# StefanSko/mcmc-db

Hardware: AMD Instinct MI355X
Metric: validated param-draws/sec (higher is better)
Workload: dtype f64; 1 GPU; single posteriordb-shaped model, 4x10000x100 synthetic draws per GPU (BASELINE config 1; AR(1) chains, ties and a shifted chain; SURVEY 8(d) C1); layout=pcn, statistics=mean,std,q5,q50,q95,split_rhat,ess_bulk,ess_tail

## Files before the change

mcmc-db_amd/csrc/mcr_kernels.hpp:

```cpp
#pragma once
#include <type_traits>
#include "mcr_device.hpp"
#include "mcr_sortnet.h"

namespace mcr {

enum ResField {
    R_MEAN = 0, R_STD, R_MEDIAN, R_RHAT, R_RHAT_BULK, R_RHAT_TAIL, R_ESS_BULK, R_ESS_TAIL,
    R_LAG_BULK, R_LAG_TAIL, R_BAD, R_Q0
};

#ifndef MCR_WCOMB
#define MCR_WCOMB 1
#endif
constexpr bool kWriteCombine = MCR_WCOMB != 0;

struct QArgs {
    int nq;
    i64 lo[32];
    double g[32];
    const void* xt = nullptr;
    int xf32 = 0;
};

// ... 194 lines not shown
        const bool sw = k[b] < k[a];                                        \
        const double lo = sw ? k[b] : k[a], hi = sw ? k[a] : k[b];          \
        const u32 ilo = sw ? ix[b] : ix[a], ihi = sw ? ix[a] : ix[b];       \
        k[a] = lo; k[b] = hi; ix[a] = ilo; ix[b] = ihi;                     \
    }
    if constexpr (VT == 16) { MCR_NET16(MCR_CE) } else { MCR_NET8(MCR_CE) }
#undef MCR_CE
}

#ifndef MCR_TILE_DPP_LEVELS
#define MCR_TILE_DPP_LEVELS 3
#endif

__device__ __forceinline__ u32 select_by_mask(u32 a, u32 b, unsigned long long m)
{
    u32 r;
    asm("v_cndmask_b32_e64 %0, %1, %2, %3" : "=v"(r) : "v"(a), "v"(b), "s"(m));
    return r;
}
__device__ __forceinline__ double select_by_mask(double a, double b, unsigned long long m)
{
    return __hiloint2double((int)select_by_mask((u32)__double2hiint(a), (u32)__double2hiint(b), m),
                            (int)select_by_mask((u32)__double2loint(a), (u32)__double2loint(b), m));
}

template <int CTRL, bool MIRROR, unsigned long long MIN_LANES>
__device__ __forceinline__ void lane_pair_stage(double (&k)[16], u32 (&ix)[16])
{
    auto exchange = [](double& own, u32& own_i, double o, u32 oi) {
        const unsigned long long lt = __builtin_amdgcn_ballot_w64(o < own), gt = __builtin_amdgcn_ballot_w64(own < o);
        const unsigned long long take = (lt & MIN_LANES) | (gt & ~MIN_LANES);
        own = select_by_mask(own, o, take);
        own_i = select_by_mask(own_i, oi, take);
    };
#pragma unroll
    for (int r = 0; r < (MIRROR ? 8 : 16); ++r) {
        const int s = MIRROR ? 15 - r : r;
        const double o_r = dpp_f64<CTRL>(k[s]);
        const u32 oi_r = dpp_u32<CTRL>(ix[s]);
        if (MIRROR) {
            const double o_s = dpp_f64<CTRL>(k[r]);
            const u32 oi_s = dpp_u32<CTRL>(ix[r]);
            exchange(k[s], ix[s], o_s, oi_s);
        }
        exchange(k[r], ix[r], o_r, oi_r);
    }
}

__device__ __forceinline__ void lane_bitonic_merge16(double (&k)[16], u32 (&ix)[16])
{
#define MCR_CE(a, b)                                                        \
    {                                                                       \
        const bool sw = k[b] < k[a];                                        \
        const double lo = sw ? k[b] : k[a], hi = sw ? k[a] : k[b];          \
        const u32 ilo = sw ? ix[b] : ix[a], ihi = sw ? ix[a] : ix[b];       \
        k[a] = lo; k[b] = hi; ix[a] = ilo; ix[b] = ihi;                     \
    }
    MCR_BITONIC16(MCR_CE)
#undef MCR_CE
}

__device__ __forceinline__ void lane_merge_levels_16_to_64(double (&k)[16], u32 (&ix)[16])
{
    constexpr unsigned long long kEvenLanes = 0x5555555555555555ull, kLowPairs = 0x3333333333333333ull;
    lane_pair_stage<0xB1, true, kEvenLanes>(k, ix);
    lane_bitonic_merge16(k, ix);
    lane_pair_stage<0x1B, true, kLowPairs>(k, ix);
    lane_pair_stage<0xB1, false, kEvenLanes>(k, ix);
    lane_bitonic_merge16(k, ix);
#if MCR_TILE_DPP_LEVELS >= 3
    constexpr unsigned long long kLowQuads = 0x0F0F0F0F0F0F0F0Full;
    lane_pair_stage<0x141, true, kLowQuads>(k, ix);
    lane_pair_stage<0x4E, false, kLowPairs>(k, ix);
    lane_pair_stage<0xB1, false, kEvenLanes>(k, ix);
    lane_bitonic_merge16(k, ix);
#endif
}

template <int VT>
__device__ __forceinline__ void serial_merge(const double* skey, int a0, int na, int b0, int nb, int ai,
                                             int bi, int nout, double (&k)[VT], int (&src)[VT])
{
    int pa = a0 + ai, pb = b0 + bi;
    const int ea = a0 + na, eb = b0 + nb;
    double ak = skey[pos16(pa)], bk = skey[pos16(pb)];
#pragma unroll
    for (int i = 0; i < VT; ++i) {
        if (i < nout) {
            const bool takeA = (pb >= eb) | ((pa < ea) & !(bk < ak));
            k[i] = takeA ? ak : bk;
            src[i] = takeA ? pa : pb;
            pa += takeA ? 1 : 0;
            pb += takeA ? 0 : 1;
            const int pn = takeA ? pa : pb;
            const double nv = skey[pos16(pn)];
            ak = takeA ? nv : ak;
            bk = takeA ? bk : nv;
        } else {
            src[i] = 0;
        }
    }
}

#ifndef MCR_TILE_REC
#define MCR_TILE_REC 1
#endif
#if MCR_TILE_REC == 0
#define MCR_TILE_PAIRS_INLINE __forceinline__
#else
#define MCR_TILE_PAIRS_INLINE __noinline__
#endif

template <typename IdxT> constexpr size_t sort_lds_bytes(int T) { return (size_t)T * (8 + sizeof(IdxT)); }

template <int NT, int VT, typename IdxT, typename XT>
__device__ MCR_TILE_PAIRS_INLINE void tile_sort_pairs(const XT* __restrict__ X, i64 M,
                                                      double* __restrict__ keys, IdxT* __restrict__ idx,
                                                      double* __restrict__ part, int ntiles,
                                                      double* __restrict__ samp)
{
    constexpr int T = NT * VT;
    extern __shared__ __attribute__((aligned(16))) char smem[];
    double* skey = reinterpret_cast<double*>(smem);
    IdxT* sidx = reinterpret_cast<IdxT*>(skey + T);
    double* red = skey;

    const int tid = threadIdx.x, tile = blockIdx.x;
    const i64 p = blockIdx.y;
    const i64 base = (i64)tile * T;
    const int count = (int)((M - base < (i64)T) ? M - base : (i64)T);
    const XT* src = X + p * M + base;

    const bool full = count == T;
    double k[VT];
    u32 ix[VT];
    double bad = 0.0;
    auto load = [&](auto full_c) {
        constexpr bool FULL = decltype(full_c)::value;
#pragma unroll
        for (int i = 0; i < VT; ++i) {
            const int e = i * NT + tid;
            const bool live = FULL || e < count;
            const double v = (double)src[FULL ? e : min(e, count - 1)];
            k[i] = live ? v : INFINITY;
            ix[i] = live ? (u32)(base + e) : 0xFFFFFFFFu;
            bad += (live && !isfinite(v)) ? 1.0 : 0.0;
        }
    };
    if (full) load(std::true_type{}); else load(std::false_type{});
    thread_sort<VT>(k, ix);
    constexpr bool kLaneLevels = MCR_TILE_DPP_LEVELS >= 2 && VT == 16;
    if constexpr (kLaneLevels) lane_merge_levels_16_to_64(k, ix);
#pragma unroll
    for (int i = 0; i < VT; ++i) {
        const int e = tid * VT + i;
        skey[pos16(e)] = k[i];
        sidx[posi(e)] = (IdxT)ix[i];
    }
    __syncthreads();

    for (int coop = kLaneLevels ? (MCR_TILE_DPP_LEVELS >= 3 ? 16 : 8) : 2; coop <= NT; coop <<= 1) {
        const int first = tid & ~(coop - 1);
        const int run = VT * (coop >> 1);
        const int a0 = first * VT, b0 = a0 + run;
        const int diag = VT * (tid - first);
        auto A = [&](int i) { return skey[pos16(a0 + i)]; };
        auto B = [&](int j) { return skey[pos16(b0 + j)]; };
        const int ai = merge_path32(A, run, B, run, diag);
        int srcs[VT];
        serial_merge<VT>(skey, a0, run, b0, run, ai, diag - ai, VT, k, srcs);
#pragma unroll
        for (int i = 0; i < VT; ++i) ix[i] = sidx[posi(srcs[i])];
        __syncthreads();
#pragma unroll
        for (int i = 0; i < VT; ++i) {
            const int e = tid * VT + i;
            skey[pos16(e)] = k[i];
            sidx[posi(e)] = (IdxT)ix[i];
        }
        __syncthreads();
    }

    auto write_out = [&](auto full_c) {
        constexpr bool FULL = decltype(full_c)::value;
#pragma nounroll
        for (int e = tid; e < (FULL ? T : count); e += NT) {
            keys[p * M + base + e] = skey[pos16(e)];
            idx[p * M + base + e] = sidx[posi(e)];
        }
    };
    if (full) write_out(std::true_type{}); else write_out(std::false_type{});
    if (samp != nullptr && tid < T / 64) {
        const int e = 64 * tid + 63;
        samp[(p * ntiles + tile) * (T / 64) + tid] = (e < count) ? skey[pos16(e)] : INFINITY;
    }
    __syncthreads();
    double s1 = 0.0, s2 = 0.0, e1 = 0.0, mt = 0.0;
    auto moments = [&](auto full_c) {
        constexpr bool FULL = decltype(full_c)::value;
        const int nlive = count - tid * VT;
#pragma unroll
        for (int i = 0; i < VT; ++i) s1 += (FULL || i < nlive) ? k[i] : 0.0;
        s1 = block_sum<NT>(s1, red);
        mt = s1 / (double)count;
#pragma unroll
        for (int i = 0; i < VT; ++i) { const double d = (FULL || i < nlive) ? k[i] - mt : 0.0; s2 = fma(d, d, s2); e1 += d; }
    };
    if (full) moments(std::true_type{}); else moments(std::false_type{});
    block_sum3<NT>(s2, e1, bad, red);
    if (tid == 0) store_slice_moments(part + (p * ntiles + tile) * kMomRec, mt, e1, s2, bad, (double)count);
}

#ifndef MCR_TILE_REC_MINMAX
#define MCR_TILE_REC_MINMAX 1
#endif
template <typename R> __device__ __forceinline__ R rec_pad();
template <> __device__ __forceinline__ u64 rec_pad<u64>() { return kRecPad; }
template <> __device__ __forceinline__ double rec_pad<double>() { return INFINITY; }

__device__ __forceinline__ void rec_ce(u64& a, u64& b)
{
    const bool sw = b < a;
    const u64 lo = sw ? b : a, hi = sw ? a : b;
    a = lo; b = hi;
}
__device__ __forceinline__ void rec_ce(double& a, double& b)
{
#if MCR_TILE_REC_MINMAX
    double lo, hi;
    asm("v_min_f64 %0, %1, %2" : "=v"(lo) : "v"(a), "v"(b));
    asm("v_max_f64 %0, %1, %2" : "=v"(hi) : "v"(a), "v"(b));
    a = lo; b = hi;
#else
    const bool sw = b < a;
    const double lo = sw ? b : a, hi = sw ? a : b;
    a = lo; b = hi;
#endif
}

template <int VT, typename R>
__device__ __forceinline__ void thread_sort_rec(R (&r)[VT])
{
    static_assert(VT == 16 || VT == 8, "sorting networks exist for 16 and 8 items per lane");
#define MCR_CE(a, b) rec_ce(r[a], r[b]);
    if constexpr (VT == 16) { MCR_NET16(MCR_CE) } else { MCR_NET8(MCR_CE) }
#undef MCR_CE
}

template <int CTRL>
__device__ __forceinline__ u64 dpp_rec(u64 v)
{
    return ((u64)dpp_u32<CTRL>((u32)(v >> 32)) << 32) | (u64)dpp_u32<CTRL>((u32)v);
}
template <int CTRL>
__device__ __forceinline__ double dpp_rec(double v) { return dpp_f64<CTRL>(v); }
__device__ __forceinline__ u64 select_by_mask(u64 a, u64 b, unsigned long long m)
{
    return ((u64)select_by_mask((u32)(a >> 32), (u32)(b >> 32), m) << 32) | (u64)select_by_mask((u32)a, (u32)b, m);
}

template <int CTRL, bool MIRROR, unsigned long long MIN_LANES, typename R>
__device__ __forceinline__ void lane_pair_stage_rec(R (&r)[16])
{
    auto exchange = [](R& own, R o) {
        const unsigned long long lt = __builtin_amdgcn_ballot_w64(o < own), gt = __builtin_amdgcn_ballot_w64(own < o);
        own = select_by_mask(own, o, (lt & MIN_LANES) | (gt & ~MIN_LANES));
    };
#pragma unroll
    for (int i = 0; i < (MIRROR ? 8 : 16); ++i) {
        const int s = MIRROR ? 15 - i : i;
        const R o_i = dpp_rec<CTRL>(r[s]);
        if (MIRROR) {
            const R o_s = dpp_rec<CTRL>(r[i]);
            exchange(r[s], o_s);
        }
        exchange(r[i], o_i);
    }
}

template <typename R>
__device__ __forceinline__ void lane_bitonic_merge16_rec(R (&r)[16])
{
#define MCR_CE(a, b) rec_ce(r[a], r[b]);
    MCR_BITONIC16(MCR_CE)
#undef MCR_CE
}

template <typename R>
__device__ __forceinline__ void lane_merge_levels_rec(R (&r)[16])
{
    constexpr unsigned long long kEvenLanes = 0x5555555555555555ull, kLowPairs = 0x3333333333333333ull,
                                 kLowQuads = 0x0F0F0F0F0F0F0F0Full;
    lane_pair_stage_rec<0xB1, true, kEvenLanes>(r);
    lane_bitonic_merge16_rec(r);
    lane_pair_stage_rec<0x1B, true, kLowPairs>(r);
    lane_pair_stage_rec<0xB1, false, kEvenLanes>(r);
    lane_bitonic_merge16_rec(r);
    lane_pair_stage_rec<0x141, true, kLowQuads>(r);
    lane_pair_stage_rec<0x4E, false, kLowPairs>(r);
    lane_pair_stage_rec<0xB1, false, kEvenLanes>(r);
    lane_bitonic_merge16_rec(r);
}

template <int VT, int LIM = 0, typename R>
__device__ __forceinline__ void serial_merge_rec(const R* srec, int a0, int na, int b0, int nb, int ai, int bi,
                                                 int nout, R (&out)[VT])
{
    int pa = a0 + ai, pb = b0 + bi;
    const int ea = a0 + na, eb = b0 + nb;
    auto slot = [](int e) { return pos16(LIM > 0 ? min(e, LIM) : e); };
    R ar = srec[slot(pa)], br = srec[slot(pb)];
#pragma unroll
    for (int i = 0; i < VT; ++i) {
        if (i < nout) {
            const bool takeA = (pb >= eb) | ((pa < ea) & !(br < ar));
            out[i] = takeA ? ar : br;
            pa += takeA ? 1 : 0;
            pb += takeA ? 0 : 1;
            const int pn = takeA ? pa : pb;
            const R nv = srec[slot(pn)];
            ar = takeA ? nv : ar;
            br = takeA ? br : nv;
        } else {
            out[i] = rec_pad<R>();
        }
    }
}

template <int NT, int VT, typename IdxT, typename XT>
__global__ __launch_bounds__(NT) __attribute__((amdgpu_waves_per_eu(4))) void k_tile_sort(const XT* __restrict__ X, i64 M,
                                                  double* __restrict__ keys, IdxT* __restrict__ idx,
                                                  double* __restrict__ part, int ntiles,
                                                  double* __restrict__ samp, unsigned* __restrict__ fallbacks)
{
#if MCR_TILE_REC == 0
    tile_sort_pairs<NT, VT, IdxT, XT>(X, M, keys, idx, part, ntiles, samp);
#else
    constexpr int T = NT * VT;
    constexpr u32 kSlotMask = 0xFFFu;
    static_assert(T <= 4096, "a record has 12 bits for the tile slot");
    extern __shared__ __attribute__((aligned(16))) char smem[];
    double* srec = reinterpret_cast<double*>(smem);
    unsigned short* slow = reinterpret_cast<unsigned short*>(srec + T);
    IdxT* sidx = reinterpret_cast<IdxT*>(srec + T);
    double* red = srec;

    const int tid = threadIdx.x, tile = blockIdx.x;
    const i64 p = blockIdx.y;
    const i64 base = (i64)tile * T;
    const int count = (int)((M - base < (i64)T) ? M - base : (i64)T);
    const XT* src = X + p * M + base;
    const bool full = count == T;
    const int nlive = count - tid * VT;

    double r[VT];
    double bad = 0.0;
    auto load = [&](auto full_c) {
        constexpr bool FULL = decltype(full_c)::value;
        XT v[VT];
#pragma unroll
        for (int i = 0; i < VT; ++i) {
            const int e = i * NT + tid;
            v[i] = src[FULL ? e : min(e, count - 1)];
        }
#pragma unroll
        for (int i = 0; i < VT; ++i) {
            const int e = i * NT + tid;
            const bool live = FULL || e < count;
            const double d = (double)v[i];
            const bool fin = isfinite(d);
            bad += (live && !fin) ? 1.0 : 0.0;
            const u32 lo = (u32)__double2loint(d), hi = (u32)__double2hiint(d);
            if (live) slow[e] = (unsigned short)(lo & kSlotMask);
            const double rec = __hiloint2double((int)(fin ? hi : 0u), (int)((lo & ~kSlotMask) | (u32)e));
            r[i] = live ? rec : INFINITY;
        }
    };
    if (full) load(std::true_type{}); else load(std::false_type{});
    thread_sort_rec<VT>(r);
    static_assert(MCR_TILE_DPP_LEVELS == 0 || MCR_TILE_DPP_LEVELS >= 3,
                  "the record sort has all three register levels or none: build MCR_TILE_DPP_LEVELS=2 with MCR_TILE_REC=0");
    constexpr bool kLaneLevels = MCR_TILE_DPP_LEVELS >= 3 && VT == 16;
    if constexpr (kLaneLevels) lane_merge_levels_rec(r);
#pragma unroll
    for (int i = 0; i < VT; ++i) srec[pos16(tid * VT + i)] = r[i];
    __syncthreads();
    for (int coop = kLaneLevels ? 16 : 2; coop <= NT; coop <<= 1) {
        const int first = tid & ~(coop - 1);
        const int run = VT * (coop >> 1);
        const int a0 = first * VT, b0 = a0 + run;
        const int diag = VT * (tid - first);
        auto A = [&](int i) { return srec[pos16(a0 + i)]; };
        auto B = [&](int j) { return srec[pos16(b0 + j)]; };
        const int ai = merge_path32(A, run, B, run, diag);
        serial_merge_rec<VT>(srec, a0, run, b0, run, ai, diag - ai, VT, r);
        __syncthreads();
        if (coop < NT) {
#pragma unroll
            for (int i = 0; i < VT; ++i) srec[pos16(tid * VT + i)] = r[i];
            __syncthreads();
        }
    }

    double k[VT];
    u32 slot[VT];
    bool viol = false;
    auto rebuild = [&](auto full_c) {
        constexpr bool FULL = decltype(full_c)::value;
#pragma unroll
        for (int i = 0; i < VT; ++i) {
            const u32 lo = (u32)__double2loint(r[i]);
            slot[i] = lo & kSlotMask;
            const double key = __hiloint2double(__double2hiint(r[i]), (int)((lo & ~kSlotMask) | (u32)slow[slot[i]]));
            k[i] = (FULL || i < nlive) ? key : INFINITY;
        }
    };
    if (full) rebuild(std::true_type{}); else rebuild(std::false_type{});
#pragma unroll
    for (int i = 0; i + 1 < VT; ++i) viol |= k[i + 1] < k[i];
    constexpr int NW = NT / kWave;
    const int lane = tid & (kWave - 1), wave = tid / kWave;
    const double next_first = dpp_f64<0x130>(k[0]);
    viol |= lane + 1 < kWave && next_first < k[VT - 1];
    int* wflag = reinterpret_cast<int*>(srec + 2 * NW);
    const bool wave_viol = __builtin_amdgcn_ballot_w64(viol) != 0;
    if (lane == 0) { srec[wave] = k[0]; wflag[wave] = wave_viol ? 1 : 0; }
    if (lane == kWave - 1) srec[NW + wave] = k[VT - 1];
    __syncthreads();
    bool fall = MCR_TILE_REC == 2;
#pragma unroll
    for (int w = 0; w < NW; ++w) {
        fall |= wflag[w] != 0;
        if (w + 1 < NW) fall |= srec[w + 1] < srec[NW + w];
    }
    __syncthreads();
    if (fall) {
        if (tid == 0 && fallbacks != nullptr) atomicAdd(fallbacks, 1u);
        tile_sort_pairs<NT, VT, IdxT, XT>(X, M, keys, idx, part, ntiles, samp);
        return;
    }
#pragma unroll
    for (int i = 0; i < VT; ++i) {
        srec[pos16(tid * VT + i)] = k[i];
        sidx[posi(tid * VT + i)] = (IdxT)((u32)base + slot[i]);
    }
    __syncthreads();

    auto write_out = [&](auto full_c) {
        constexpr bool FULL = decltype(full_c)::value;
#pragma nounroll
        for (int e = tid; e < (FULL ? T : count); e += NT) {
            keys[p * M + base + e] = srec[pos16(e)];
            idx[p * M + base + e] = sidx[posi(e)];
        }
    };
    if (full) write_out(std::true_type{}); else write_out(std::false_type{});
    if (samp != nullptr && tid < T / 64) {
        const int e = 64 * tid + 63;
        samp[(p * ntiles + tile) * (T / 64) + tid] = (e < count) ? srec[pos16(e)] : INFINITY;
    }
    __syncthreads();
    double s1 = 0.0, s2 = 0.0, e1 = 0.0, mt = 0.0;
    auto moments = [&](auto full_c) {
        constexpr bool FULL = decltype(full_c)::value;
#pragma unroll
        for (int i = 0; i < VT; ++i) s1 += (FULL || i < nlive) ? k[i] : 0.0;
        s1 = block_sum<NT>(s1, red);
        mt = s1 / (double)count;
#pragma unroll
        for (int i = 0; i < VT; ++i) { const double d = (FULL || i < nlive) ? k[i] - mt : 0.0; s2 = fma(d, d, s2); e1 += d; }
    };
    if (full) moments(std::true_type{}); else moments(std::false_type{});
    block_sum3<NT>(s2, e1, bad, red);
    if (tid == 0) store_slice_moments(part + (p * ntiles + tile) * kMomRec, mt, e1, s2, bad, (double)count);
#endif
}

template <int NT, int VT>
__device__ __forceinline__ void scatter_codes_by_line(u32* __restrict__ zrow, i64 M, int total, const u32 (&hcode)[VT],
                                                      const u32 (&hpos)[VT], u32* cnt_code, unsigned short* spos, u32* swt)
{
    constexpr int kMaxLines = 2048, PER = kMaxLines / NT > 0 ? kMaxLines / NT : 1;
    static_assert(NT * PER >= kMaxLines, "every line counter has an owner in the scan");
    const int tid = threadIdx.x;
    const int nlines = (int)((M + 31) >> 5);
    u32* scnt = cnt_code;
    u32* scode = cnt_code + 2112;
    __syncthreads();
    for (int i = tid; i <= nlines; i += NT) scnt[i] = 0u;
    __syncthreads();
    u32 rk[VT];
#pragma unroll
    for (int i = 0; i < VT; ++i) rk[i] = (tid * VT + i < total) ? atomicAdd(&scnt[hpos[i] >> 5], 1u) : 0u;
    __syncthreads();
    {
        u32 c[PER], tsum = 0;
#pragma unroll
        for (int j = 0; j < PER; ++j) { const int q = tid * PER + j; c[j] = (q < nlines) ? scnt[q] : 0u; tsum += c[j]; }
        u32 wtot;
        const u32 wex = wave_excl_scan_u32(tsum, wtot);
        if ((tid & 63) == 0) swt[tid >> 6] = wtot;
        __syncthreads();
        u32 base = wex;
        for (int w = 0; w < (tid >> 6); ++w) base += swt[w];
#pragma unroll
        for (int j = 0; j < PER; ++j) { const int q = tid * PER + j; if (q < nlines) scnt[q] = base; base += c[j]; }
    }
    __syncthreads();
#pragma unroll
    for (int i = 0; i < VT; ++i) {
        if (tid * VT + i < total) {
            const u32 slot = min(scnt[hpos[i] >> 5] + rk[i], (u32)(NT * VT - 1));
            scode[slot] = hcode[i];
            spos[slot] = (unsigned short)hpos[i];
        }
    }
    __syncthreads();
    for (int e = tid; e < total; e += NT) zrow[spos[e]] = scode[e];
}

template <int NT, int VT, class KF>
__device__ __forceinline__ void block_tie_runs(KF key_at, int total, int* wsh, int (&rs)[VT], int (&re)[VT])
{
    constexpr int NW = NT / kWave;
    const int tid = threadIdx.x, lane = tid & 63, w = tid >> 6;
    const int base = tid * VT;
    bool h[VT];
    auto prev = key_at((base > 0 && base - 1 < total) ? base - 1 : 0);
    int cur = -1, first = 0x7fffffff;
#pragma unroll
    for (int i = 0; i < VT; ++i) {
        const int g = base + i;
        const auto kv = key_at(g < total ? g : 0);
        h[i] = (g == 0) || (g >= total) || (prev != kv);
        if (h[i]) { cur = g; if (first == 0x7fffffff) first = g; }
        rs[i] = cur;
        prev = kv;
    }
    int exL, exR;
    const int incl = wave_prefix_max(cur, exL);
    const int rinc = wave_suffix_min(first, exR);
    __syncthreads();
    if (lane == 63) wsh[w] = incl;
    if (lane == 0) wsh[NW + w] = rinc;
    __syncthreads();
    int carryL = -1, carryR = total;
#pragma unroll
    for (int ww = 0; ww < NW; ++ww) {
        if (ww < w) carryL = max(carryL, wsh[ww]);
        if (ww > w) carryR = min(carryR, wsh[NW + ww]);
    }
    carryL = max(carryL, exL);
    carryR = min(carryR, exR);
    if (carryR > total) carryR = total;
    int nxt = carryR;
#pragma unroll
    for (int i = VT - 1; i >= 0; --i) {
        re[i] = nxt;
        if (h[i]) nxt = base + i;
        if (rs[i] < 0) rs[i] = carryL;
    }
    __syncthreads();
}

__device__ __forceinline__ bool sign_bit_set(double v) { return __double_as_longlong(v) < 0; }
__device__ __forceinline__ bool sign_bit_set(float v) { return __float_as_int(v) < 0; }
template <typename T>
__device__ __noinline__ unsigned wave_zero_signs(const T* __restrict__ x, i64 M, i64 t0, i64 t1)
{
    constexpr int U = 8;
    const int lane = threadIdx.x & 63;
    i64 seen = 0, t = (t0 >= 0) ? t0 : t1;
    unsigned out = 0;
    for (i64 b = 0; b < M; b += 64 * U) {
        T v[U];
#pragma unroll
        for (int u = 0; u < U; ++u) {
            const i64 i = b + u * 64 + lane;
            v[u] = (i < M) ? x[i] : (T)1;
        }
        i64 c = 0;
#pragma unroll
        for (int u = 0; u < U; ++u) c += (i64)__popcll(__ballot(v[u] == (T)0));
        if (seen + c <= t) { seen += c; continue; }
#pragma unroll
        for (int u = 0; u < U; ++u) {
            const unsigned long long zm = __ballot(v[u] == (T)0), nm = __ballot(v[u] == (T)0 && sign_bit_set(v[u]));
            const i64 cu = (i64)__popcll(zm);
            while (seen + cu > t) {
                unsigned long long m = zm;
                for (i64 j = seen; j < t; ++j) m &= m - 1;
                const bool neg = (nm & m & (~m + 1ull)) != 0;
                if (t == t1) return out | (neg ? 2u : 0u);
                out |= neg ? 1u : 0u;
                t = t1;
            }
            seen += cu;
        }
    }
    return out;
}

template <typename KT>
__device__ __forceinline__ i64 wave_order_stats(const KT* __restrict__ k, i64 M, const QArgs& q, bool write,
                                                double* __restrict__ res, i64 P, i64 p, double& med_out)
{
#pragma clang fp contract(off)
    const int lane = threadIdx.x & 63;
    if (write && lane < q.nq) {
        const int j = lane;
        const i64 lo = q.lo[j], hi = (lo + 1 < M) ? lo + 1 : M - 1;
        const double a = sorted_key(k, lo), b = sorted_key(k, hi), d = b - a, g = q.g[j];
        res[(R_Q0 + j) * P + p] = (g >= 0.5) ? b - d * (1.0 - g) : a + d * g;
    }
    const double below = (M >= 2) ? sorted_key(k, M / 2 - 1) : -INFINITY, at = sorted_key(k, M / 2);
    double med = (M & 1) ? at : (below + at) / 2.0;
    const bool zero_med = write && q.xt != nullptr && at == 0.0 && ((M & 1) || below == 0.0);
    if (write && lane == 0 && !zero_med) res[R_MEDIAN * P + p] = med;
    i64 lo = 0, hi = M;
    if (below < med && !(at < med)) {
        if (!zero_med) { med_out = med; return M / 2; }
        lo = hi = M / 2;
    }
    while (lo < hi) {
        const i64 step = (hi - lo + 63) / 64;
        const i64 pos = lo + step * (lane + 1) - 1;
        const bool less = (pos < hi) && (sorted_key(k, pos) < med);
        const i64 cnt = (i64)__popcll(__ballot(less));
        const i64 nhi = lo + step * (cnt + 1) - 1;
        lo += step * cnt;
        hi = (nhi < hi) ? nhi : hi;
    }
    if (zero_med) {
        const i64 r = M / 2 - lo;
        const i64 t0 = (M & 1) ? -1 : r - 1;
        const unsigned sg = q.xf32 ? wave_zero_signs(reinterpret_cast<const float*>(q.xt) + p * M, M, t0, r)
                                   : wave_zero_signs(reinterpret_cast<const double*>(q.xt) + p * M, M, t0, r);
        const bool neg = (M & 1) ? (sg & 2u) != 0 : sg == 3u;
        med = neg ? -0.0 : 0.0;
        if (lane == 0) res[R_MEDIAN * P + p] = med;
    }
    med_out = med;
    return lo;
}

template <int NT, int VT, bool FOLD, typename IdxT, typename KT = double>
__global__ __launch_bounds__(NT) void k_merge(const KT* __restrict__ kin, const IdxT* __restrict__ iin,
                                              double* __restrict__ kout, IdxT* __restrict__ iout, i64 M,
                                              i64 R, double* __restrict__ res, i64 P,
                                              QArgs q, u32* __restrict__ z, const i64* __restrict__ split_in)
{
    constexpr int OBS = NT * VT;
    constexpr int OB = FOLD ? OBS - 64 : OBS;
    extern __shared__ __attribute__((aligned(16))) char smem[];
    double* skey = reinterpret_cast<double*>(smem);
    IdxT* sidx = reinterpret_cast<IdxT*>(skey + OBS);
    i64* sh = FOLD ? reinterpret_cast<i64*>(skey + OB) : reinterpret_cast<i64*>(sidx + OBS);

    const int tid = threadIdx.x;
    i64 p = blockIdx.y;
    int blk = blockIdx.x;
    if (FOLD) {
        if (!xcd_map(P, (int)((M + OB - 1) / OB), p, blk)) return;
    }
    const i64 o0 = (i64)blk * OB;
    if (o0 >= M) return;
    const KT* kp = kin + p * M;
    const IdxT* ip = iin + p * M;
    auto KEY = [&](i64 g) -> double { return sorted_key(kp, g); };
    auto POS = [&](i64 g) -> u32 {
        if constexpr (sizeof(KT) == 8 && !__is_same(KT, double)) return (u32)kp[g]; else return (u32)ip[g];
    };

    i64 abase, na, bbase, nb, d0;
    double med = 0.0;
    if (!FOLD) {
        const i64 pb = (o0 / (2 * R)) * (2 * R);
        abase = pb;
        na = (M - pb < R) ? M - pb : R;
        bbase = pb + na;
        nb = (M - bbase < R) ? M - bbase : R;
        d0 = o0 - pb;
    } else {
        if (split_in != nullptr) {
            if (tid == 0) { sh[0] = split_in[p]; reinterpret_cast<double*>(sh)[1] = res[R_MEDIAN * P + p]; }
        } else if (tid < 64) {
            double m_;
            const i64 s_ = wave_order_stats(kp, M, q, blk == 0, res, P, p, m_);
            if (tid == 0) { sh[0] = s_; reinterpret_cast<double*>(sh)[1] = m_; }
        }
        __syncthreads();
        const i64 s = sh[0];
        med = reinterpret_cast<double*>(sh)[1];
        __syncthreads();
        abase = s - 1;
        na = s;
        bbase = s;
        nb = M - s;
        d0 = o0;
    }
    const i64 tot = na + nb;
    const i64 d1 = (d0 + OB < tot) ? d0 + OB : tot;
// ... 583 lines not shown
```

mcmc-db_amd/csrc/mcr_sort32.hpp:

```cpp
#pragma once
#include "mcr_kernels.hpp"

namespace mcr {

__device__ __forceinline__ u32 rec_key(u64 r) { return (u32)(r >> 32); }
__device__ __forceinline__ u32 rec_pos(u64 r) { return (u32)r; }


constexpr size_t rec_lds_bytes(int T) { return (size_t)(T + 2) * 8; }

template <int NT, int VT>
__global__ __launch_bounds__(NT) void k_tile_sort32(const float* __restrict__ X, i64 M, u64* __restrict__ recs,
                                                    double* __restrict__ part, int ntiles, double* __restrict__ samp)
{
    constexpr int T = NT * VT;
    extern __shared__ __attribute__((aligned(16))) char smem[];
    u64* srec = reinterpret_cast<u64*>(smem);
    double* red = reinterpret_cast<double*>(smem);

    const int tid = threadIdx.x, tile = blockIdx.x;
    const i64 p = blockIdx.y;
    const i64 base = (i64)tile * T;
    const int count = (int)((M - base < (i64)T) ? M - base : (i64)T);
    const float* src = X + p * M + base;

    const bool full = count == T;
    u64 r[VT];
    double bad = 0.0;
    auto load = [&](auto full_c) {
        constexpr bool FULL = decltype(full_c)::value;
#pragma unroll
        for (int i = 0; i < VT; ++i) {
            const int e = i * NT + tid;
            const bool live = FULL || e < count;
            const float v = src[FULL ? e : min(e, count - 1)];
            bad += (live && !isfinite(v)) ? 1.0 : 0.0;
            r[i] = live ? (((u64)f32_key(v) << 32) | (u64)(u32)(base + e)) : kRecPad;
        }
    };
    if (full) load(std::true_type{}); else load(std::false_type{});
    thread_sort_rec<VT>(r);
    constexpr bool kLaneLevels = MCR_TILE_DPP_LEVELS >= 3 && VT == 16;
    if constexpr (kLaneLevels) lane_merge_levels_rec(r);
#pragma unroll
    for (int i = 0; i < VT; ++i) srec[pos16(tid * VT + i)] = r[i];
    __syncthreads();

    for (int coop = kLaneLevels ? 16 : 2; coop <= NT; coop <<= 1) {
        const int first = tid & ~(coop - 1);
        const int run = VT * (coop >> 1);
        const int a0 = first * VT, b0 = a0 + run;
        const int diag = VT * (tid - first);
        auto A = [&](int i) { return srec[pos16(a0 + i)]; };
        auto B = [&](int j) { return srec[pos16(b0 + j)]; };
        const int ai = merge_path32(A, run, B, run, diag);
        serial_merge_rec<VT, T - 1>(srec, a0, run, b0, run, ai, diag - ai, VT, r);
        __syncthreads();
#pragma unroll
        for (int i = 0; i < VT; ++i) srec[pos16(tid * VT + i)] = r[i];
        __syncthreads();
    }
    auto write_out = [&](auto full_c) {
        constexpr bool FULL = decltype(full_c)::value;
#pragma nounroll
        for (int e = tid; e < (FULL ? T : count); e += NT) recs[p * M + base + e] = srec[pos16(e)];
    };
    if (full) write_out(std::true_type{}); else write_out(std::false_type{});
    if (samp != nullptr && tid < T / 64) {
        const int e = 64 * tid + 63;
        samp[(p * ntiles + tile) * (T / 64) + tid] = (e < count) ? key_value(rec_key(srec[pos16(e)])) : INFINITY;
    }
    __syncthreads();
    double s1 = 0.0, s2 = 0.0, e1 = 0.0, mt = 0.0;
    auto moments = [&](auto full_c) {
        constexpr bool FULL = decltype(full_c)::value;
        const int nlive = count - tid * VT;
#pragma unroll
        for (int i = 0; i < VT; ++i) s1 += (FULL || i < nlive) ? key_value(rec_key(r[i])) : 0.0;
        s1 = block_sum<NT>(s1, red);
        mt = s1 / (double)count;
#pragma unroll
        for (int i = 0; i < VT; ++i) { const double d = (FULL || i < nlive) ? key_value(rec_key(r[i])) - mt : 0.0; s2 = fma(d, d, s2); e1 += d; }
    };
    if (full) moments(std::true_type{}); else moments(std::false_type{});
    block_sum3<NT>(s2, e1, bad, red);
    if (tid == 0) store_slice_moments(part + (p * ntiles + tile) * kMomRec, mt, e1, s2, bad, (double)count);
}

template <int NT, int VT>
__global__ __launch_bounds__(NT) void k_merge32(const u64* __restrict__ rin, u64* __restrict__ rout, i64 M, i64 R)
{
    constexpr int OB = NT * VT;
    extern __shared__ __attribute__((aligned(16))) char smem[];
    u64* srec = reinterpret_cast<u64*>(smem);
    __shared__ i64 sh[2];
    const int tid = threadIdx.x;
    const i64 p = blockIdx.y;
    const i64 o0 = (i64)blockIdx.x * OB;
    if (o0 >= M) return;
    const u64* rp = rin + p * M;
    const i64 pb = (o0 / (2 * R)) * (2 * R);
    const i64 abase = pb, na = (M - pb < R) ? M - pb : R;
    const i64 bbase = pb + na, nb = (M - bbase < R) ? M - bbase : R;
    const i64 d0 = o0 - pb, tot = na + nb;
    const i64 d1 = (d0 + OB < tot) ? d0 + OB : tot;
    auto GA = [&](i64 i) { return rp[abase + i]; };
    auto GB = [&](i64 j) { return rp[bbase + j]; };
    if (tid < 64) { const i64 r0 = merge_path_wave(GA, na, GB, nb, d0); if (tid == 0) sh[0] = r0; }
    else if (tid < 128) { const i64 r1 = merge_path_wave(GA, na, GB, nb, d1); if (tid == 64) sh[1] = r1; }
    __syncthreads();
    const i64 ai0 = sh[0], ai1 = sh[1], bi0 = d0 - ai0;
    const int ca = (int)(ai1 - ai0), cb = (int)((d1 - ai1) - bi0);
    const int total = ca + cb;
    {
        u64 gr[VT];
#pragma unroll
        for (int j = 0; j < VT; ++j) {
            const int e = j * NT + tid;
            const i64 g = (e < ca) ? abase + ai0 + e : bbase + bi0 + (e - ca);
            gr[j] = rp[(e < total) ? g : 0];
        }
#pragma unroll
        for (int j = 0; j < VT; ++j) {
            const int e = j * NT + tid;
            if (e < total) srec[pos16(e)] = gr[j];
        }
    }
    __syncthreads();
    const int diag = (tid * VT < total) ? tid * VT : total;
    const int nout = (total - diag < VT) ? total - diag : VT;
    auto A = [&](int i) { return srec[pos16(i)]; };
    auto B = [&](int j) { return srec[pos16(ca + j)]; };
    const int ai = merge_path32(A, ca, B, cb, diag);
    u64 r[VT];
    serial_merge_rec<VT>(srec, 0, ca, ca, cb, ai, diag - ai, nout, r);
    __syncthreads();
#pragma unroll
    for (int i = 0; i < VT; ++i)
        if (i < nout) srec[pos16(diag + i)] = r[i];
    __syncthreads();
    for (int e = tid; e < total; e += NT) rout[p * M + o0 + e] = srec[pos16(e)];
}

template <int NT, int VT>
__global__ __launch_bounds__(NT) void k_bucket_merge32(const u64* __restrict__ rin, u64* __restrict__ rout, i64 M,
                                                       int k, int B, const u32* __restrict__ cut,
                                                       const u32* __restrict__ boff, u32* __restrict__ z, i64 P, i64 R)
{
    constexpr int T = NT * VT;
    static_assert(T == 4096, "the partition bound of k_splitters assumes 4096-slot buckets");
    extern __shared__ __attribute__((aligned(16))) char smem[];
    u64* srec = reinterpret_cast<u64*>(smem);
    int* sst = reinterpret_cast<int*>(srec + T + 2);
    int* spl = sst + kBkLen;
    int* sps = sst + kBkSrc;
    int* sext = sst + kBkExt;
    i64* sedge = reinterpret_cast<i64*>(sst + kBkEdge);
    u64* sne = reinterpret_cast<u64*>(sst + kBkNext);
    static_assert(2 * (NT / kWave) <= 4 * kMaxBucketTiles, "the tie-run scratch takes the neighbours' place");

    const int tid = threadIdx.x;
    i64 p;
    int b;
    if (!xcd_map(P, B, p, b)) return;
    const u64* rp = rin + p * M;
    const u32* c0 = cut + (p * (B + 1) + b) * k;
    const u32* c1 = c0 + k;
    if (k < 1 || k > kMaxBucketTiles) return;
    if (tid < kWave) bucket_piece_table(c0, c1, k, sst, spl, sps);
    __syncthreads();
    const int padded = sst[k];
    const int total = (int)(boff[p * (B + 1) + b + 1] - boff[p * (B + 1) + b]);
    const i64 obase = boff[p * (B + 1) + b];
    if (padded > T - 64 || total < 0 || total > padded || obase + total > M) return;
    const int ne_lane = tid - (T - 64 - (VT - 1) * NT);
    bool ne_there = false;
    i64 ne_g = 0;
    if (ne_lane >= 0) ne_g = bucket_neighbour(ne_lane, k, R, M, spl, sps, ne_there);
    const bool is_ne = ne_lane >= 0 && ne_lane < 2 * k;
    u64 ne = 0;
    {
        const int lane = tid & 63, wv = tid >> 6;
        u32 my_g = 0; int my_n = 0;
        if ((lane & 15) < VT) {
            const int e0 = (lane & 15) * NT + 64 * wv + 16 * (lane >> 4);
            if (e0 < padded) {
                int t = 0;
#pragma unroll
                for (int step = 8; step > 0; step >>= 1)
                    if (t + step < k && e0 >= sst[t + step]) t += step;
                const int o = e0 - sst[t];
                my_n = spl[t] - o;
                my_g = (u32)((i64)t * R) + (u32)sps[t] + (u32)o;
            }
        }
        u64 gr[VT];
#pragma unroll
        for (int j = 0; j < VT; ++j) {
            const int within = lane & 15;
            const u32 g0 = (u32)row_lane((int)my_g, j);
            const int n = row_lane(my_n, j);
            const bool live = within < n;
            i64 g = live ? (i64)(g0 + (u32)within) : 0;
            if (j == VT - 1) g = is_ne ? ne_g : g;
            const u64 r = rp[g];
            gr[j] = live ? r : kRecPad;
            if (j == VT - 1) ne = r;
        }
#pragma unroll
        for (int j = 0; j < VT; ++j) {
            const int e = j * NT + tid;
            if (e < padded) srec[pos16(e)] = gr[j];
        }
    }
    if (is_ne) sne[ne_lane] = ne_there ? (u64)rec_key(ne) : ~0ull;
    wait_loads();
    __syncthreads();
    const int chunk0 = tid * VT;
    int mypiece = 0;
#pragma unroll
    for (int step = 8; step > 0; step >>= 1)
        if (mypiece + step < k && chunk0 >= sst[mypiece + step]) mypiece += step;
    for (int w = 1; w < k; w <<= 1) {
        u64 r[VT];
        bool moved = false;
        if (chunk0 < padded) {
            const int ra = mypiece & ~(2 * w - 1);
            const int a0 = sst[ra];
            const int a1 = sst[(ra + w < k) ? ra + w : k];
            const int b1 = sst[(ra + 2 * w < k) ? ra + 2 * w : k];
            const int na = a1 - a0, nb = b1 - a1, diag = chunk0 - a0;
            moved = nb > 0;
            if (moved) {
                auto A = [&](int i) { return srec[pos16(a0 + i)]; };
                auto Bf = [&](int j) { return srec[pos16(a1 + j)]; };
                const int ai = merge_path32(A, na, Bf, nb, diag);
                serial_merge_rec<VT>(srec, a0, na, a1, nb, ai, diag - ai, VT, r);
            }
        }
        __syncthreads();
        if (moved) {
#pragma unroll
            for (int i = 0; i < VT; ++i) srec[pos16(chunk0 + i)] = r[i];
        }
        __syncthreads();
    }
    for (int e = tid; e < total; e += NT) rout[p * M + obase + e] = srec[pos16(e)];
    if (z == nullptr || total == 0) return;
    if (tid < 4) sedge[tid] = 0;
    const u32 kfirst = rec_key(srec[pos16(0)]), klast = rec_key(srec[pos16(total - 1)]);
    if (tid < kWave) {
        const int t = (tid < k) ? tid : k - 1;
        const bool e0 = tid < k && sne[t] == (u64)kfirst;
        const bool e1 = tid < k && sne[k + t] == (u64)klast;
        const bool a0 = __ballot(e0) != 0, a1 = __ballot(e1) != 0;
        if (tid == 0) { sext[0] = a0; sext[1] = a1; }
    }
    __syncthreads();
    const bool ext0 = sext[0] != 0, ext1 = sext[1] != 0;
    if ((ext0 || ext1) && tid < 2 * k) {
        const int t = tid % k, which = tid / k;
        const u32 v = which ? klast : kfirst;
        const i64 tbase = (i64)t * R;
        const int cnt = (int)((M - tbase < R) ? M - tbase : R);
        const u64* a = rp + tbase;
        int lo = 0, hi = cnt;
        while (lo < hi) { const int m = (lo + hi) >> 1; if (rec_key(a[m]) < v) lo = m + 1; else hi = m; }
        const int lb = lo;
        hi = cnt;
        while (lo < hi) { const int m = (lo + hi) >> 1; if (!(v < rec_key(a[m]))) lo = m + 1; else hi = m; }
        atomicAdd(reinterpret_cast<unsigned long long*>(&sedge[2 * which]), (unsigned long long)lb);
        atomicAdd(reinterpret_cast<unsigned long long*>(&sedge[2 * which + 1]), (unsigned long long)lo);
    }
    __syncthreads();
    int rs[VT], re[VT];
    block_tie_runs<NT, VT>([&](int g) { return rec_key(srec[pos16(g)]); }, total, sst + kBkNext, rs, re);
#pragma unroll
    for (int i = 0; i < VT; ++i) {
        const int e = tid * VT + i;
        if (e < total) {
            const u64 r = srec[pos16(e)];
            i64 gs = obase + rs[i], ge = obase + re[i];
            if (ext0 && rec_key(r) == kfirst) gs = sedge[0];
            if (ext1 && rec_key(r) == klast) ge = sedge[3];
            z[p * M + min(rec_pos(r), (u32)(M - 1))] = (u32)(gs + ge);
        }
    }
}

}
```

Baseline: 27.14 billion param-draws/s.

## Merge tile runs as bitonic sequences with mirrored second-run stores

Each thread stores its sorted run of records so that the second run of every merge pair sits in reverse order in shared memory. The merge then walks inward from both ends of the bitonic sequence, which removes the end-of-run bounds checks and turns the serial merge into min/max plus a ballot-driven index update written in inline asm. The mirrored store folds the reversal into the 16-slot XOR swizzle, so this path requires VT == 16 and hand-written GCN assembly for carry-based pointer advance. The float32 sort kernel loses its old non-mirrored fallback and always uses the new path.

```diff
diff --git a/mcmc-db_amd/csrc/mcr_kernels.hpp b/mcmc-db_amd/csrc/mcr_kernels.hpp
--- a/mcmc-db_amd/csrc/mcr_kernels.hpp
+++ b/mcmc-db_amd/csrc/mcr_kernels.hpp
@@ -520,14 +520,13 @@
     lane_bitonic_merge16_rec(r);
 }
 
-template <int VT, int LIM = 0, typename R>
+template <int VT, typename R>
 __device__ __forceinline__ void serial_merge_rec(const R* srec, int a0, int na, int b0, int nb, int ai, int bi,
                                                  int nout, R (&out)[VT])
 {
     int pa = a0 + ai, pb = b0 + bi;
     const int ea = a0 + na, eb = b0 + nb;
-    auto slot = [](int e) { return pos16(LIM > 0 ? min(e, LIM) : e); };
-    R ar = srec[slot(pa)], br = srec[slot(pb)];
+    R ar = srec[pos16(pa)], br = srec[pos16(pb)];
 #pragma unroll
     for (int i = 0; i < VT; ++i) {
         if (i < nout) {
@@ -536,13 +535,79 @@
             pa += takeA ? 1 : 0;
             pb += takeA ? 0 : 1;
             const int pn = takeA ? pa : pb;
-            const R nv = srec[slot(pn)];
+            const R nv = srec[pos16(pn)];
             ar = takeA ? nv : ar;
             br = takeA ? br : nv;
         } else {
             out[i] = rec_pad<R>();
         }
     }
+}
+
+#ifndef MCR_TILE_MERGE_ENDS
+#define MCR_TILE_MERGE_ENDS 1
+#endif
+template <int VT>
+__device__ __forceinline__ void serial_merge_ends(const double* srec, int left, int right, double (&out)[VT])
+{
+    double u = srec[pos16(left)], v = srec[pos16(right)];
+    unsigned long long vright = ~0ull;
+    u32 nl = (u32)left + 1u, nr = (u32)right - 1u;
+#pragma unroll
+    for (int i = 0; i < VT; ++i) {
+        double lo, hi, vnext = 0.0;
+        if (i + 1 < VT) {
+            vright ^= __builtin_amdgcn_ballot_w64(u < v);
+            vnext = srec[pos16((int)select_by_mask(nl, nr, vright))];
+            unsigned long long carry;
+            asm volatile("v_subb_co_u32_e64 %0, %2, %0, -1, %3\n\t"
+                         "v_subb_co_u32_e64 %1, %2, %1, 0, %3"
+                         : "+v"(nl), "+v"(nr), "=&s"(carry) : "s"(vright));
+        }
+        asm volatile("v_min_f64 %0, %1, %2" : "=v"(lo) : "v"(u), "v"(v));
+        if (i + 1 < VT) {
+            asm volatile("v_max_f64 %0, %1, %2" : "=v"(hi) : "v"(u), "v"(v));
+            u = hi;
+        }
+        out[i] = lo;
+        v = vnext;
+    }
+}
+
+template <int VT>
+__device__ __forceinline__ void serial_merge_ends(const u64* srec, int left, int right, u64 (&out)[VT])
+{
+    u64 u = srec[pos16(left)], v = srec[pos16(right)];
+    unsigned long long vright = ~0ull;
+    u32 nl = (u32)left + 1u, nr = (u32)right - 1u;
+#pragma unroll
+    for (int i = 0; i < VT; ++i) {
+        const unsigned long long lt = __builtin_amdgcn_ballot_w64(u < v);
+        u64 vnext = 0;
+        if (i + 1 < VT) {
+            vright ^= lt;
+            vnext = srec[pos16((int)select_by_mask(nl, nr, vright))];
+            unsigned long long carry;
+            asm volatile("v_subb_co_u32_e64 %0, %2, %0, -1, %3\n\t"
+                         "v_subb_co_u32_e64 %1, %2, %1, 0, %3"
+                         : "+v"(nl), "+v"(nr), "=&s"(carry) : "s"(vright));
+        }
+        out[i] = select_by_mask(v, u, lt);
+        if (i + 1 < VT) u = select_by_mask(u, v, lt);
+        v = vnext;
+    }
+}
+
+template <typename R>
+__device__ __forceinline__ void store_runs_mirrored(R* srec, int tid, int half, const R (&r)[16])
+{
+    static_assert(sizeof(R) == 8, "records are 8 bytes");
+    const bool odd = (tid & half) != 0;
+    const int tm = odd ? tid ^ (half - 1) : tid;
+    const int c = (tm & 15) ^ (odd ? 15 : 0);
+    const int b8 = (tm * 16 + c) << 3;
+#pragma unroll
+    for (int i = 0; i < 16; ++i) *reinterpret_cast<R*>(reinterpret_cast<char*>(srec) + (b8 ^ (i << 3))) = r[i];
 }
 
 template <int NT, int VT, typename IdxT, typename XT>
@@ -600,22 +665,38 @@
                   "the record sort has all three register levels or none: build MCR_TILE_DPP_LEVELS=2 with MCR_TILE_REC=0");
     constexpr bool kLaneLevels = MCR_TILE_DPP_LEVELS >= 3 && VT == 16;
     if constexpr (kLaneLevels) lane_merge_levels_rec(r);
-#pragma unroll
-    for (int i = 0; i < VT; ++i) srec[pos16(tid * VT + i)] = r[i];
-    __syncthreads();
-    for (int coop = kLaneLevels ? 16 : 2; coop <= NT; coop <<= 1) {
+    constexpr int kFirstCoop = kLaneLevels ? 16 : 2;
+#if MCR_TILE_MERGE_ENDS
+    static_assert(VT == 16, "the mirrored store folds 15 - i into the 16-slot swizzle");
+    auto store_runs = [&](int half) { store_runs_mirrored(srec, tid, half, r); };
+#else
+    auto store_runs = [&](int) {
+#pragma unroll
+        for (int i = 0; i < VT; ++i) srec[pos16(tid * VT + i)] = r[i];
+    };
+#endif
+    store_runs(kFirstCoop >> 1);
+    __syncthreads();
+    for (int coop = kFirstCoop; coop <= NT; coop <<= 1) {
         const int first = tid & ~(coop - 1);
         const int run = VT * (coop >> 1);
-        const int a0 = first * VT, b0 = a0 + run;
+        const int a0 = first * VT;
         const int diag = VT * (tid - first);
         auto A = [&](int i) { return srec[pos16(a0 + i)]; };
+#if MCR_TILE_MERGE_ENDS
+        const int last = a0 + 2 * run - 1;
+        auto B = [&](int j) { return srec[pos16(last - j)]; };
+        const int ai = merge_path32(A, run, B, run, diag);
+        serial_merge_ends<VT>(srec, a0 + ai, last - (diag - ai), r);
+#else
+        const int b0 = a0 + run;
         auto B = [&](int j) { return srec[pos16(b0 + j)]; };
         const int ai = merge_path32(A, run, B, run, diag);
         serial_merge_rec<VT>(srec, a0, run, b0, run, ai, diag - ai, VT, r);
+#endif
         __syncthreads();
         if (coop < NT) {
-#pragma unroll
-            for (int i = 0; i < VT; ++i) srec[pos16(tid * VT + i)] = r[i];
+            store_runs(coop);
             __syncthreads();
         }
     }
diff --git a/mcmc-db_amd/csrc/mcr_sort32.hpp b/mcmc-db_amd/csrc/mcr_sort32.hpp
--- a/mcmc-db_amd/csrc/mcr_sort32.hpp
+++ b/mcmc-db_amd/csrc/mcr_sort32.hpp
@@ -42,22 +42,24 @@
     thread_sort_rec<VT>(r);
     constexpr bool kLaneLevels = MCR_TILE_DPP_LEVELS >= 3 && VT == 16;
     if constexpr (kLaneLevels) lane_merge_levels_rec(r);
-#pragma unroll
-    for (int i = 0; i < VT; ++i) srec[pos16(tid * VT + i)] = r[i];
-    __syncthreads();
-
-    for (int coop = kLaneLevels ? 16 : 2; coop <= NT; coop <<= 1) {
+    constexpr int kFirstCoop = kLaneLevels ? 16 : 2;
+    static_assert(VT == 16, "the mirrored store folds 15 - i into the 16-slot swizzle");
+    auto store_runs = [&](int half) { store_runs_mirrored(srec, tid, half, r); };
+    store_runs(kFirstCoop >> 1);
+    __syncthreads();
+
+    for (int coop = kFirstCoop; coop <= NT; coop <<= 1) {
         const int first = tid & ~(coop - 1);
         const int run = VT * (coop >> 1);
-        const int a0 = first * VT, b0 = a0 + run;
+        const int a0 = first * VT;
         const int diag = VT * (tid - first);
         auto A = [&](int i) { return srec[pos16(a0 + i)]; };
-        auto B = [&](int j) { return srec[pos16(b0 + j)]; };
+        const int last = a0 + 2 * run - 1;
+        auto B = [&](int j) { return srec[pos16(last - j)]; };
         const int ai = merge_path32(A, run, B, run, diag);
-        serial_merge_rec<VT, T - 1>(srec, a0, run, b0, run, ai, diag - ai, VT, r);
-        __syncthreads();
-#pragma unroll
-        for (int i = 0; i < VT; ++i) srec[pos16(tid * VT + i)] = r[i];
+        serial_merge_ends<VT>(srec, a0 + ai, last - (diag - ai), r);
+        __syncthreads();
+        store_runs(coop);
         __syncthreads();
     }
     auto write_out = [&](auto full_c) {
```

After: 27.42 billion param-draws/s (median of 6 runs). +1.0%, better.
